# isarandi/metro-pose3d

Measured on AMD Instinct MI355X. Metric: crops/sec (256x256, RN50 stride16), higher is better.
Workload: dtype f16

## Files before the change

### metro_pose3d_amd/csrc/conv_b1.hip

```cpp
#ifndef METRO_WT_STORES
#define METRO_WT_STORES 1
#endif
#include "metro_common.h"
#include "gfx950_prims.h"

namespace metro {

namespace b1 {
constexpr int NPROD = 8, NCONS = 4, NT = 64 * (NPROD + NCONS), TN = 64, K = 64, CB = 256, C2 = 64, NBUF = 3;
constexpr int X_BYTES = TN * 128;
constexpr int OUT_ROW = CB * 2 + 16;
constexpr int OUT_BYTES = TN * OUT_ROW;
constexpr int W1S_ROW = CB * 2 + 16;
static_assert(48 * W1S_ROW <= OUT_BYTES, "W1's stage must fit the second output tile");
template <bool REB>
struct Lay {
    static constexpr int NIN = REB ? 3 : 2;
    static constexpr int X_OFF = 0;
    static constexpr int OUT_OFF = NBUF * NIN * X_BYTES;
    static constexpr int PAR_OFF = OUT_OFF + 2 * OUT_BYTES;
    static constexpr int B3 = 0, BSC = 1024, BB = 2048, B2 = 3072, PRO = 3328, SC2 = 3584, SH2 = 4096, PAR_BYTES = 4608;
    static constexpr int W1T_OFF = PAR_OFF + PAR_BYTES;
    static constexpr int LDS = W1T_OFF + 8 * 64 * 16;
};
// ... 140 lines not shown
#pragma unroll
                    for (int kk = 0; kk < 4; ++kk)
#pragma unroll
                        for (int p = 0; p < 2; ++p) {
                            const half8_t bb = *reinterpret_cast<const half8_t*>(xs + 2 * X_BYTES + p * 4096 + (boff0 ^ (kk << 5)));
                            acc[p] = __builtin_amdgcn_mfma_f32_32x32x16_f16(wbf[kk], bb, acc[p], 0, 0, 0);
                        }
#pragma unroll
                    for (int q = 0; q < 4; ++q) {
                        const floatx4 bv = *reinterpret_cast<const floatx4*>(bias_b_l + wave * 32 + 8 * q + 4 * frag_half);
#pragma unroll
                        for (int p = 0; p < 2; ++p) xsum[p][q] = bias_cvt(acc[p], q, bv) + xsum[p][q];
                    }
                }
#pragma unroll
                for (int p = 0; p < 2; ++p)
#pragma unroll
                    for (int e = 0; e < 16; ++e) acc[p][e] = 0.f;
#pragma unroll
                for (int kk = 0; kk < 4; ++kk)
#pragma unroll
                    for (int p = 0; p < 2; ++p) {
                        const half8_t bf = *reinterpret_cast<const half8_t*>(xs + p * 4096 + (boff0 ^ (kk << 5)));
                        acc[p] = __builtin_amdgcn_mfma_f32_32x32x16_f16(wf[kk], bf, acc[p], 0, 0, 0);
                    }
#pragma unroll
                for (int q = 0; q < 4; ++q) {
                    const int col = wave * 32 + 8 * q + 4 * frag_half;
#pragma unroll
                    for (int p = 0; p < 2; ++p)
                        *reinterpret_cast<half4_t*>(ot + (p * 32 + frag_row) * OUT_ROW + col * 2) = bias_cvt(acc[p], q, b3_r[q]) + xsum[p][q];
                }
            }
            slot = slot == 2 ? 0 : slot + 1;
        }
    } else {
        half8_t w2r[3][8];
        wait_vm_and_barrier<0>();
#pragma unroll
        for (int mt = 0; mt < 3; ++mt)
#pragma unroll
            for (int ks = 0; ks < 8; ++ks) {
                w2r[mt][ks] = *reinterpret_cast<const half8_t*>(smem + L::OUT_OFF + OUT_BYTES + (mt * 16 + (lane & 15)) * W1S_ROW + ks * 64 + (lane >> 4) * 16);
                asm volatile("" : "+v"(w2r[mt][ks]));
            }
        const int wb = wave - NPROD;
        const int px = wb * 16 + (lane & 15), kg = lane >> 4;
        for (int j = 0; j <= T; ++j) {
            wait_lgkm_and_barrier();
            if (j == 0) continue;
            const int tile = t0 + (j - 1) * G;
            const char* ot = smem + L::OUT_OFF + ((j - 1) & 1) * OUT_BYTES;
            const size_t m = (size_t)tile * TN + px;
            bool sub_ok = false;
            size_t sub_row = 0;
            if constexpr (OUTM == 2) {
                const int hw = a.h_out * a.w_out;
                const int m0 = tile * TN + wb * 16;
                const int img = m0 / hw, rem = m0 - img * hw;
                const int hr = (rem >> a.lw_out) - a.sub_off;
                const int wo = ((rem & (a.w_out - 1)) + (lane & 15)) - a.sub_off;
                sub_ok = hr >= 0 && (hr & 1) == 0 && (hr >> 1) < a.h_sub && wo >= 0 && (wo & 1) == 0 && (wo >> 1) < a.w_sub;
                sub_row = ((size_t)img * a.h_sub + (hr >> 1)) * a.w_sub + (wo >> 1);
            }
            floatx4 dacc[4];
#pragma unroll
            for (int mt = 0; mt < 4; ++mt) dacc[mt] = floatx4{0.f, 0.f, 0.f, 0.f};
#pragma unroll
            for (int ks = 0; ks < 8; ++ks) {
                const uint4 v = *reinterpret_cast<const uint4*>(ot + px * OUT_ROW + ks * 64 + kg * 16);
                if constexpr (OUTM == 0) store_out16(a.out + m * CB + ks * 32 + kg * 8, v);
                if constexpr (OUTM == 2) {
                    if (sub_ok) store_out16(a.out_sub + sub_row * CB + ks * 32 + kg * 8, v);
                }
                const half8_t s = *reinterpret_cast<const half8_t*>(par + L::SC2 + (ks * 32 + kg * 8) * 2);
                const half8_t b = *reinterpret_cast<const half8_t*>(par + L::SH2 + (ks * 32 + kg * 8) * 2);
                half8_t pv = *reinterpret_cast<const half8_t*>(&v);
                pv = relu(pv * s + b);
                const half8_t w3 = *reinterpret_cast<const half8_t*>(smem + L::W1T_OFF + (ks * 64 + lane) * 16);
#pragma unroll
                for (int mt = 0; mt < 3; ++mt) dacc[mt] = __builtin_amdgcn_mfma_f32_16x16x32_f16(w2r[mt][ks], pv, dacc[mt], 0, 0, 0);
                dacc[3] = __builtin_amdgcn_mfma_f32_16x16x32_f16(w3, pv, dacc[3], 0, 0, 0);
            }
#pragma unroll
            for (int mt = 0; mt < 4; ++mt) {
                const int co = mt * 16 + kg * 4;
                const floatx4 bv = *reinterpret_cast<const floatx4*>(par + L::B2 + co * 4);
                half4_t hv;
#pragma unroll
                for (int e = 0; e < 4; ++e) hv[e] = (half_t)relu(dacc[mt][e] + bv[e]);
                *reinterpret_cast<half4_t*>(a.out2 + m * C2 + co) = hv;
            }
        }
    }
}

static thread_local int g_b1_force_classic = 0;
void conv_b1_set_form(int classic) { g_b1_force_classic = classic; }
bool classic_forms_forced() { return g_b1_force_classic != 0; }

bool conv_b1_chain_preferred() {
    static const int enabled = tuning_knob("METRO_B1_SPLIT", 1);
    return enabled != 0 && g_b1_force_classic == 0;
}

template <bool REB, int OUTM>
static int launch_b1(B1Args a, hipStream_t stream) {
    if (note_kernel("conv_b1_chain<%s%s>", REB ? "rebuild" : "projsc", OUTM == 1 ? ",noout" : OUTM == 2 ? ",subout" : ""))
        return METRO_OK;
    auto kern = conv_b1_chain_kernel<REB, OUTM>;
    constexpr int lds = b1::Lay<REB>::LDS;
    a.n_tiles = a.m_total / b1::TN;
    static PerDeviceInt cap;
    int grid_cap = 0;
    if (const int st = ensure_dyn_lds_and_grid_cap(reinterpret_cast<const void*>(kern), b1::NT, lds, cap, "conv_b1_chain", 1, &grid_cap))
        return st;
    const int grid = a.n_tiles < grid_cap ? a.n_tiles : grid_cap;
    hipLaunchKernelGGL(kern, dim3(grid), dim3(b1::NT), lds, stream, a);
    return launch_status("conv_b1_chain");
}

int launch_conv_b1_chain(const MetroConvDesc& d, const void* in, const void* w, const float* bias, void* out, hipStream_t stream,
                         const ConvFused& f) {
    const ConvFuse2& f2 = f.next;
    const ConvProjSc& psc = f.psc;
    const ConvRebuild& rb = f.rb;
    B1Args a;
    a.in = static_cast<const half_t*>(in); a.w = static_cast<const half_t*>(w); a.bias = bias;
    a.x_sc = static_cast<const half_t*>(psc.x); a.w_sc = static_cast<const half_t*>(psc.w_sc); a.bias_sc = psc.bias_sc;
    a.pro_scale = static_cast<const half_t*>(psc.pro_scale); a.pro_shift = static_cast<const half_t*>(psc.pro_shift);
    a.in_b = static_cast<const half_t*>(rb.t2_prev); a.w_b = static_cast<const half_t*>(rb.w3_prev); a.bias_b = rb.bias3_prev;
    a.w2 = static_cast<const half_t*>(f2.w2); a.bias2 = f2.bias2;
    a.scale2 = static_cast<const half_t*>(f2.scale2); a.shift2 = static_cast<const half_t*>(f2.shift2);
    a.out = static_cast<half_t*>(out); a.out_sub = static_cast<half_t*>(rb.out_sub); a.out2 = static_cast<half_t*>(f2.out2);
    a.m_total = d.n * d.h_out * d.w_out; a.n_tiles = 0;
    a.h_out = d.h_out; a.w_out = d.w_out; a.lw_out = 0;
    while ((1 << a.lw_out) < d.w_out) ++a.lw_out;
    a.sub_off = rb.sub_off; a.h_sub = rb.h_sub; a.w_sub = rb.w_sub;
    if (f.form == ConvForm::NextRebuild) return rb.out_mode == 2 ? launch_b1<true, 2>(a, stream) : launch_b1<true, 0>(a, stream);
    return rb.out_mode == 1 ? launch_b1<false, 1>(a, stream) : launch_b1<false, 0>(a, stream);
}

}
```

### metro_pose3d_amd/csrc/conv_pw64.hip

```cpp
#include <cstdlib>
#include <type_traits>

#ifndef METRO_WT_STORES
#define METRO_WT_STORES 1
#endif
#include "metro_common.h"
#include "gfx950_prims.h"

namespace metro {

struct Pw64Args {
    const half_t* in;
    const half_t* w;
    const float* bias;
    const half_t* pro_scale;
    const half_t* pro_shift;
    const half_t* residual;
    half_t* out;
    const half_t* w2;
    const float* bias2;
    const half_t* scale2;
    const half_t* shift2;
    half_t* out2;
    const half_t* x_sc;
    const half_t* w_sc;
    const float* bias_sc;
    const half_t* in_b;
    const half_t* w_b;
    const float* bias_b;
    half_t* out_sub;
    int sub_off, h_sub, w_sub, lw_out;
    int m_total, n_tiles;
    int c_out;
    int res_stride, res_off, res_h, res_w, h_out, w_out;
};

namespace pw {
constexpr int NW = 8, NT = 512;
template <int K, int WM, int CB = 256>
struct Lay {
    static constexpr int WN = NW / WM;
    static constexpr int NI = CB / 32 / WM;
    static constexpr int TN = 32 * WN;
    static constexpr int KS = K / 64;
    static constexpr int SL_BYTES = TN * 128;
    static constexpr int X_BYTES = KS * SL_BYTES;
    static constexpr int XI = X_BYTES / 1024 / NW;
    static constexpr int CPR = CB / 8;
    static constexpr int RI = TN * CPR / NT;
    static constexpr int OUT_ROW = CB * 2 + 16;
    static constexpr int OUT_BYTES = TN * OUT_ROW;
    static constexpr int RES_BYTES = TN * CB * 2;
    static constexpr int C2 = CB == 512 ? 128 : 64;
    static constexpr int BIAS2_OFF = CB * 4, PRO_OFF = BIAS2_OFF + 512, BSC_OFF = PRO_OFF + 4 * K, BB_OFF = BSC_OFF + 1024;
    static constexpr int PAR_BYTES = BB_OFF + 1024;
    static constexpr int X_OFF = 0;
    static constexpr int OUT_OFF = X_OFF + 2 * X_BYTES;
    static constexpr int PAR_OFF = OUT_OFF + OUT_BYTES;
    static constexpr int RES_OFF = PAR_OFF + PAR_BYTES;
    static_assert(X_BYTES % (1024 * NW) == 0, "input tile must split evenly over the waves");
    static_assert(NI >= 1 && RI >= 1 && (TN * CPR) % NT == 0, "tile / thread mismatch");
};
template <int K, int WM, bool RES, int MODE2, bool PSC = false, int CB = 256, bool REB = false>
constexpr int lds_bytes() {
    return Lay<K, WM, CB>::RES_OFF + (RES ? 2 * Lay<K, WM, CB>::RES_BYTES : PSC ? (REB ? 4 : 2) * Lay<K, WM, CB>::X_BYTES
                                      : (MODE2 == 1 && K > 64) ? Lay<K, WM, CB>::C2 * (2 * K + 16) + Lay<K, WM, CB>::TN * (2 * Lay<K, WM, CB>::C2 + 16) : 0);
}
}

template <int BASE, int MAXX>
__device__ __forceinline__ void pw_wait_vm_plus(int extra) {
    if constexpr (MAXX == 0) {
        wait_vm<BASE>();
    } else {
        if (extra >= MAXX) wait_vm<BASE + MAXX>();
        else pw_wait_vm_plus<BASE, MAXX - 1>(extra);
    }
}
__device__ __forceinline__ void pw_wait_lgkm2(half8_t& r, half8_t& r2, int n) {
    switch (n) {
        case 0: asm volatile("s_waitcnt lgkmcnt(0)" : "+v"(r), "+v"(r2)); break;
        case 2: asm volatile("s_waitcnt lgkmcnt(2)" : "+v"(r), "+v"(r2)); break;
        case 4: asm volatile("s_waitcnt lgkmcnt(4)" : "+v"(r), "+v"(r2)); break;
        default: asm volatile("s_waitcnt lgkmcnt(6)" : "+v"(r), "+v"(r2)); break;
    }
}

// ... 80 lines not shown
    constexpr bool W2_LDS = MODE2 == 1 && K > 64;
    constexpr bool PREPASS = PRO && W2_LDS;
    constexpr int W2_ROW = 2 * K + 16;
    constexpr int W2_OFF = RES_OFF;
    constexpr int O2_ROW = 2 * C2 + 16, O2_OFF = W2_OFF + C2 * W2_ROW;
    half8_t w2f[MODE2 == 1 && !W2_LDS ? KK : 1];
    if constexpr (MODE2 == 1 && !W2_LDS) {
        if (wave < 4) {
#pragma unroll
            for (int kk = 0; kk < KK; ++kk)
                w2f[kk] = *reinterpret_cast<const half8_t*>(a.w2 + (size_t)(wm * 32 + frag_row) * K + kk * 16 + frag_half * 8);
        }
    }
    if constexpr (W2_LDS) {
        for (int c = tid; c < C2 * (K / 8); c += NT) {
            const int r = c / (K / 8), q = c % (K / 8);
            *reinterpret_cast<uint4*>(smem + W2_OFF + r * W2_ROW + q * 16) = *reinterpret_cast<const uint4*>(a.w2 + (size_t)r * K + q * 8);
        }
    }
    const char* w2l = smem + W2_OFF + (wm * 32 + frag_row) * W2_ROW + frag_half * 16;
    float* bias_l = reinterpret_cast<float*>(smem + PAR_OFF);
    float* bias2_l = reinterpret_cast<float*>(smem + PAR_OFF + L::BIAS2_OFF);
    half_t* pro_l = reinterpret_cast<half_t*>(smem + PAR_OFF + L::PRO_OFF);
    if (tid < CB) bias_l[tid] = a.bias[tid];
    if (MODE2 != 0 && tid < C2) bias2_l[tid] = a.bias2[tid];
    if ((PRO || PSC) && tid < K) { pro_l[tid] = a.pro_scale[tid]; pro_l[K + tid] = a.pro_shift[tid]; }
    float* bias_sc_l = reinterpret_cast<float*>(smem + PAR_OFF + L::BSC_OFF);
    if (PSC && tid < 256) bias_sc_l[tid] = a.bias_sc[tid];
    float* bias_b_l = reinterpret_cast<float*>(smem + PAR_OFF + L::BB_OFF);
    if (REB && tid < 256) bias_b_l[tid] = a.bias_b[tid];
    const int ch = tid & (CPR - 1);
    half8_t sc2 = {}, sh2 = {};
    if constexpr (MODE2 == 2) {
        sc2 = *reinterpret_cast<const half8_t*>(a.scale2 + ch * 8);
        sh2 = *reinterpret_cast<const half8_t*>(a.shift2 + ch * 8);
        if constexpr (!W_STAGED) {
#pragma unroll
            for (int ks = 0; ks < KS2; ++ks)
                w2r[ks] = *reinterpret_cast<const half8_t*>(a.w2 + (size_t)((wave % RG) * 16 + (lane & 15)) * CB + ks * 32 + (lane >> 4) * 8);
        }
    }

    int xrow[XI], xoff[XI];
#pragma unroll
    for (int i = 0; i < XI; ++i) {
        const int q = i * NW + wave;
        xrow[i] = (q % (TN / 8)) * 8 + (lane >> 3);
        xoff[i] = xrow[i] * K + (q / (TN / 8)) * 64 + (((lane & 7) ^ swz<64>(xrow[i])) * 8);
    }
    auto issue_tile = [&](int tile, int buf) {
        const int m0 = tile * TN;
#pragma unroll
        for (int i = 0; i < XI; ++i) {
            const half_t* xs = (m0 + xrow[i] < a.m_total) ? a.in + (size_t)m0 * K + xoff[i] : zero;
            dma16(xs, __builtin_amdgcn_readfirstlane(smem_base + X_OFF + buf * X_BYTES + (i * NW + wave) * 1024));
            if constexpr (PSC) {
                const half_t* ss = (m0 + xrow[i] < a.m_total) ? a.x_sc + (size_t)m0 * K + xoff[i] : zero;
                dma16(ss, __builtin_amdgcn_readfirstlane(smem_base + XS_OFF + buf * X_BYTES + (i * NW + wave) * 1024));
            }
            if constexpr (REB) {
                const half_t* sb = (m0 + xrow[i] < a.m_total) ? a.in_b + (size_t)m0 * K + xoff[i] : zero;
                dma16(sb, __builtin_amdgcn_readfirstlane(smem_base + XB_OFF + buf * X_BYTES + (i * NW + wave) * 1024));
            }
        }
        if constexpr (RES) {
#pragma unroll
            for (int it = 0; it < RI; ++it) {
                const int c = it * NT + tid;
                const int m = m0 + c / CPR;
                size_t rrow = m;
                if constexpr (RSUB) {
                    const int hw = a.h_out * a.w_out;
                    const int img = m / hw, rem = m - img * hw;
                    const int ho = rem / a.w_out, wo = rem - ho * a.w_out;
                    rrow = ((size_t)img * a.res_h + a.res_off + a.res_stride * ho) * a.res_w + a.res_off + a.res_stride * wo;
                }
                const half_t* rs = m < a.m_total ? a.residual + rrow * ldo + (c & (CPR - 1)) * 8 : zero;
                dma16(rs, __builtin_amdgcn_readfirstlane(smem_base + RES_OFF + buf * RES_BYTES + it * 8192 + wave * 1024));
            }
        }
    };

    issue_tile(t, 0);
    constexpr int S2 = MODE2 == 2 ? NTW : (MODE2 == 1 && K > 64) ? 1 : 4;
    constexpr int RS = OUTM == 0 ? RI : 0;
    const bool two = MODE2 == 2 || (MODE2 == 1 && (wave < 4 || K > 64));
    bool prev_full = false;
    int prev_sub = 0;
    for (int it = 0;; ++it, t += G) {
        const int buf = it & 1;
        const int m0 = t * TN;
        if (it == 0 || !prev_full) wait_vm<0>();
        else if constexpr (OUTM == 2) pw_wait_vm_plus<S2, RI>(prev_sub);
        else if (two) wait_vm<RS + S2>();
        else wait_vm<RS>();
        wait_lgkm_and_barrier();
        if (t + G < a.n_tiles) issue_tile(t + G, buf ^ 1);
        prev_full = m0 + TN <= a.m_total;

        if constexpr (PREPASS) {
            static_assert(X_BYTES / 16 == 2 * NT, "two 16-byte chunks of the input tile per thread");
            const int c8 = lane & 7, prow = (wave & 3) * 8 + (lane >> 3);
#pragma unroll
            for (int h = 0; h < 2; ++h) {
                const int sl = (wave >> 2) + 2 * h;
                half8_t* xp = reinterpret_cast<half8_t*>(smem + X_OFF + buf * X_BYTES + sl * SL_BYTES + prow * 128 + ((c8 ^ swz<64>(prow)) << 4));
                const half8_t sc = *reinterpret_cast<const half8_t*>(pro_l + sl * 64 + c8 * 8);
                const half8_t sh = *reinterpret_cast<const half8_t*>(pro_l + K + sl * 64 + c8 * 8);
                *xp = relu(*xp * sc + sh);
            }
            wait_lgkm_and_barrier();
        }
        floatx16 acc[NI], acc2, accs[NI];
#pragma unroll
        for (int e = 0; e < 16; ++e) {
#pragma unroll
            for (int i = 0; i < NI; ++i) { acc[i][e] = 0.f; accs[i][e] = 0.f; }
            acc2[e] = 0.f;
        }
        const char* xl = smem + X_OFF + buf * X_BYTES;
        const int brow = wn * 32 + frag_row;
        half4_t xprev[NI][4];
        if constexpr (REB) {
#pragma unroll
            for (int kk = 0; kk < KK; ++kk) {
                const int chunk = (kk & 3) * 2 + frag_half;
                half8_t bs = *reinterpret_cast<const half8_t*>(smem + XS_OFF + buf * X_BYTES + (kk >> 2) * SL_BYTES + brow * 128 + ((chunk ^ swz<64>(brow)) << 4));
                const half8_t s = *reinterpret_cast<const half8_t*>(pro_l + kk * 16 + frag_half * 8);
                const half8_t b = *reinterpret_cast<const half8_t*>(pro_l + K + kk * 16 + frag_half * 8);
                bs = relu(bs * s + b);
#pragma unroll
                for (int i = 0; i < NI; ++i) accs[i] = __builtin_amdgcn_mfma_f32_32x32x16_f16(wsf[i][kk], bs, accs[i], 0, 0, 0);
            }
#pragma unroll
            for (int i = 0; i < NI; ++i)
#pragma unroll
                for (int q = 0; q < 4; ++q) {
                    const floatx4 bs = *reinterpret_cast<const floatx4*>(bias_sc_l + (wm * NI + i) * 32 + 8 * q + 4 * frag_half);
#pragma unroll
                    for (int e = 0; e < 4; ++e) xprev[i][q][e] = (half_t)(accs[i][4 * q + e] + bs[e]);
                }
            floatx16 accb[NI];
#pragma unroll
            for (int i = 0; i < NI; ++i)
#pragma unroll
                for (int e = 0; e < 16; ++e) accb[i][e] = 0.f;
#pragma unroll
            for (int kk = 0; kk < KK; ++kk) {
                const int chunk = (kk & 3) * 2 + frag_half;
                const half8_t bb = *reinterpret_cast<const half8_t*>(smem + XB_OFF + buf * X_BYTES + (kk >> 2) * SL_BYTES + brow * 128 + ((chunk ^ swz<64>(brow)) << 4));
#pragma unroll
                for (int i = 0; i < NI; ++i) accb[i] = __builtin_amdgcn_mfma_f32_32x32x16_f16(wbf[i][kk], bb, accb[i], 0, 0, 0);
            }
#pragma unroll
            for (int i = 0; i < NI; ++i)
#pragma unroll
                for (int q = 0; q < 4; ++q) {
                    const floatx4 bv = *reinterpret_cast<const floatx4*>(bias_b_l + (wm * NI + i) * 32 + 8 * q + 4 * frag_half);
                    half4_t hb;
#pragma unroll
                    for (int e = 0; e < 4; ++e) hb[e] = (half_t)(accb[i][4 * q + e] + bv[e]);
                    xprev[i][q] = hb + xprev[i][q];
                }
        }
        if constexpr (PREPASS) {
            constexpr int DEPTH = 3;
            unsigned fbase[4];
// ... 95 lines not shown
#pragma unroll
                    for (int e = 0; e < 4; ++e) hs[e] = (half_t)(accs[i][4 * q + e] + bs[e]);
                    hv = hv + hs;
                }
                *reinterpret_cast<half4_t*>(ol + brow * OUT_ROW + col * 2) = hv;
            }
        }
        wait_lgkm_and_barrier();
        const char* rl = smem + RES_OFF + buf * RES_BYTES;
        int img0 = 0, rem0 = 0, now_sub = 0;
        if constexpr (OUTM == 2) {
            const int hw = a.h_out * a.w_out;
            img0 = m0 / hw;
            rem0 = m0 - img0 * hw;
        }
        uint4 vpre[OUTM == 0 ? RI : 1], rpre[OUTM == 0 && RES ? RI : 1];
        if constexpr (OUTM == 0) {
#pragma unroll
            for (int r = 0; r < RI; ++r) {
                const int idx = tid + r * NT;
                vpre[r] = *reinterpret_cast<const uint4*>(ol + (idx / CPR) * OUT_ROW + ch * 16);
                if constexpr (RES) rpre[r] = *reinterpret_cast<const uint4*>(rl + idx * 16);
            }
            __builtin_amdgcn_sched_barrier(0);
        }
        const bool inside = m0 + TN <= a.m_total;
#pragma unroll
        for (int r = 0; r < RI; ++r) {
            const int idx = tid + r * NT;
            const int prow = idx / CPR;
            const int m = m0 + prow;
            uint4 v;
            if constexpr (OUTM == 0) v = vpre[r];
            else v = *reinterpret_cast<const uint4*>(ol + prow * OUT_ROW + ch * 16);
            if constexpr (RES) {
                uint4 rv;
                if constexpr (OUTM == 0) rv = rpre[r];
                else rv = *reinterpret_cast<const uint4*>(rl + idx * 16);
                half2_t* x = reinterpret_cast<half2_t*>(&v);
                const half2_t* rr = reinterpret_cast<const half2_t*>(&rv);
#pragma unroll
                for (int e = 0; e < 4; ++e) x[e] = x[e] + rr[e];
            }
            if constexpr (OUTM == 0) {
                if (inside) store_out16(a.out + (size_t)m * ldo + ch * 8, v);
                else if (m < a.m_total) store_out16(a.out + (size_t)m * ldo + ch * 8, v);
            }
            if constexpr (OUTM == 2) {
                const int hr = ((rem0 + 16 * r) >> a.lw_out) - a.sub_off;
                if (hr >= 0 && (hr & 1) == 0 && (hr >> 1) < a.h_sub) {
                    ++now_sub;
                    const int wo = ((rem0 + prow) & (a.w_out - 1)) - a.sub_off;
                    if (wo >= 0 && (wo & 1) == 0 && (wo >> 1) < a.w_sub)
                        store_out16(a.out_sub + (((size_t)img0 * a.h_sub + (hr >> 1)) * a.w_sub + (wo >> 1)) * CB + ch * 8, v);
                }
            }
            if constexpr (MODE2 == 2) {
                half8_t p = *reinterpret_cast<const half8_t*>(&v);
                p = relu(p * sc2 + sh2);
                *reinterpret_cast<half8_t*>(ol + prow * OUT_ROW + ch * 16) = p;
            }
        }
        if constexpr (W2_LDS) {
            static_assert(TN * (C2 / 8) == NT, "one 16-byte chunk of the second output per thread");
            const int prow2 = tid / (C2 / 8), ch2 = tid % (C2 / 8);
            const uint4 v2 = *reinterpret_cast<const uint4*>(smem + O2_OFF + prow2 * O2_ROW + ch2 * 16);
            if (m0 + prow2 < a.m_total) store_out16(a.out2 + (size_t)(m0 + prow2) * C2 + ch2 * 8, v2);
        }
        if constexpr (MODE2 == 2) {
            wait_lgkm_and_barrier();
            floatx4 dacc[NTW];
#pragma unroll
            for (int j = 0; j < NTW; ++j) dacc[j] = floatx4{0.f, 0.f, 0.f, 0.f};
            const int px0 = (wave / RG) * (NTW * 16);
            const char* bl = ol + (px0 + (lane & 15)) * OUT_ROW + (lane >> 4) * 16;
#pragma unroll
            for (int ks = 0; ks < KS2; ++ks) {
#pragma unroll
                for (int j = 0; j < NTW; ++j) {
                    const half8_t bj = *reinterpret_cast<const half8_t*>(bl + j * 16 * OUT_ROW + ks * 64);
                    dacc[j] = __builtin_amdgcn_mfma_f32_16x16x32_f16(w2r[ks], bj, dacc[j], 0, 0, 0);
                }
            }
            const int co = (wave % RG) * 16 + (lane >> 4) * 4;
            const floatx4 bv = *reinterpret_cast<const floatx4*>(bias2_l + co);
#pragma unroll
            for (int j = 0; j < NTW; ++j) {
                const int m = m0 + px0 + j * 16 + (lane & 15);
                half4_t hv;
#pragma unroll
                for (int e = 0; e < 4; ++e) hv[e] = (half_t)relu(dacc[j][e] + bv[e]);
                if (m < a.m_total) *reinterpret_cast<half4_t*>(a.out2 + (size_t)m * C2 + co) = hv;
            }
        }
        prev_sub = now_sub;
        if (t + G >= a.n_tiles) break;
    }
}

static bool pw_enabled() {
    static const int v = tuning_knob("METRO_PW64", 1);
    return v != 0;
}

static bool b1_map_ok(const MetroConvDesc& d) {
    return (d.h_out * d.w_out) % 64 == 0 && d.w_out >= 16 && (d.w_out & (d.w_out - 1)) == 0;
}

bool conv_pw64_supported(const MetroConvDesc& d, const ConvFused& f) {
    if (!pw_enabled()) return false;
    if (!(d.kh == 1 && d.kw == 1 && d.stride == 1 && d.pad_top == 0 && d.pad_left == 0 && d.in_pix_stride == d.c_in &&
          d.h_in == d.h_out && d.w_in == d.w_out && d.relu == 0 && d.out_dtype == METRO_F16 && d.in_dtype == METRO_F16))
        return false;
    const bool res_plain = d.res_stride == 1 && d.res_offset == 0 && d.res_h == d.h_out && d.res_w == d.w_out;
    const bool res_sub = d.res_stride == 2 && d.res_offset >= 0 && d.res_offset + 2 * (d.h_out - 1) < d.res_h &&
                         d.res_offset + 2 * (d.w_out - 1) < d.res_w;
    if (d.has_residual && !res_plain && !(f.form == ConvForm::Plain && res_sub && d.c_in <= 128)) return false;
    switch (f.form) {
        case ConvForm::Pair: {
            static const int pair256 = tuning_knob("METRO_PW_PAIR256", 1);
            return ((d.c_in == 64 && d.c_out == 320) || (pair256 && !classic_forms_forced() && d.c_in == 256 && d.c_out == 640)) &&
                   d.has_prologue && !d.has_residual && f.pair.relu2 == 1 && 5 * f.pair.c_out2 == d.c_out && f.pair.split == 4 * f.pair.c_out2;
        }
        case ConvForm::Next: {
            static const int next128 = tuning_knob("METRO_PW_NEXT128", 1);
            return ((d.c_in == 64 && d.c_out == 256 && f.next.c2 == 64) ||
                    (next128 && d.c_in == 128 && d.c_out == 512 && res_plain && f.next.c2 == 128)) && !d.has_prologue && d.has_residual;
        }
        case ConvForm::NextProj:
        case ConvForm::NextRebuild:
            return d.c_in == 64 && d.c_out == 256 && !d.has_prologue && !d.has_residual && f.next.c2 == 64 &&
                   (f.form == ConvForm::NextProj || b1_map_ok(d));
        case ConvForm::Plain:
            break;
    }
    if (d.c_in == 64 && d.c_out == 256) return (d.has_prologue != 0) != (d.has_residual != 0);
    static const int maxk = tuning_knob("METRO_PW_MAXK", 512);
    return (d.c_in == 128 || d.c_in == 256 || d.c_in == 512) && d.c_in <= maxk && d.c_out == 4 * d.c_in &&
           !d.has_prologue && d.has_residual;
}

template <int K, int WM, bool PRO, bool RES, int MODE2, bool RSUB = false, bool PSC = false, int CB = 256, bool REB = false, int OUTM = 0>
static int launch_pw(Pw64Args a, hipStream_t stream) {
    if (note_kernel("conv_pw64<k%d,wm%d%s%s%s%s%s%s%s%s>", K, WM, CB == 512 ? ",cb512" : "", PRO ? ",pro" : "", RES ? ",res" : "",
                    MODE2 == 1 ? ",pair" : MODE2 == 2 ? ",next" : "", RSUB ? ",ressub" : "", PSC ? ",projsc" : "", REB ? ",rebuild" : "",
                    OUTM == 1 ? ",noout" : OUTM == 2 ? ",subout" : ""))
        return METRO_OK;
    auto kern = conv_pw64_kernel<K, WM, PRO, RES, MODE2, RSUB, PSC, CB, REB, OUTM>;
    constexpr int lds = pw::lds_bytes<K, WM, RES, MODE2, PSC, CB, REB>();
    a.n_tiles = (a.m_total + pw::Lay<K, WM, CB>::TN - 1) / pw::Lay<K, WM, CB>::TN;
    static PerDeviceInt cap;
    int grid_cap = 0;
    if (const int st = ensure_dyn_lds_and_grid_cap(reinterpret_cast<const void*>(kern), pw::NT, lds, cap, "conv_pw64",
                                                   tuning_knob("METRO_PW64_BPC", 0) , &grid_cap))
        return st;
    const int halves = a.c_out / CB;
    int grid = a.n_tiles * halves < grid_cap ? a.n_tiles * halves : grid_cap;
    grid -= grid % halves;
    hipLaunchKernelGGL(kern, dim3(grid), dim3(pw::NT), lds, stream, a);
    return launch_status("conv_pw64");
}

int launch_conv_pw64(const MetroConvDesc& d, const void* in, const void* w, const float* bias, const void* ps,
                     const void* pb, const void* res, void* out, hipStream_t stream, const ConvFused& f) {
    const ConvRebuild& rb = f.rb;
    if ((f.form == ConvForm::NextRebuild || (f.form == ConvForm::NextProj && rb.out_mode == 1)) && !rb.classic &&
        conv_b1_chain_preferred() && b1_map_ok(d))
        return launch_conv_b1_chain(d, in, w, bias, out, stream, f);
    Pw64Args a;
    a.in = static_cast<const half_t*>(in);
    a.w = static_cast<const half_t*>(w);
    a.bias = bias;
    a.pro_scale = static_cast<const half_t*>(ps);
    a.pro_shift = static_cast<const half_t*>(pb);
    a.residual = d.has_residual ? static_cast<const half_t*>(res) : nullptr;
// ... 46 lines not shown
```

### metro_pose3d_amd/csrc/conv_pws.hip

```cpp
#include "metro_common.h"
#include "gfx950_prims.h"

namespace metro {

struct PwsArgs {
    const half_t* in;
    const half_t* w;
    const float* bias;
    const half_t* residual;
    half_t* out;
    int m_total, n_tiles, c_out;
};

namespace pws {
constexpr int NW = 8, NT = 512, TN = 32, CB = 256, NBUF = 3;
constexpr int T_ROW = 80;
constexpr int T_BYTES = TN * T_ROW;
constexpr int R_BYTES = TN * 64;
template <int K>
struct Lay {
    static constexpr int KS = K / 64;
    static constexpr int SL_BYTES = TN * 128;
    static constexpr int X_BYTES = KS * SL_BYTES;
    static constexpr int NX = X_BYTES / 1024 / NW;
    static constexpr int X_OFF = 0;
    static constexpr int T_OFF = NBUF * X_BYTES;
    static constexpr int BIAS_OFF = T_OFF + NW * (T_BYTES + R_BYTES);
    static constexpr int LDS = BIAS_OFF + CB * 4;
    static_assert(X_BYTES % (1024 * NW) == 0, "operand tile must split evenly over the waves");
};
}

template <int K>
__global__ __launch_bounds__(pws::NT) void conv_pws_kernel(PwsArgs a) {
    using namespace pws;
    using L = Lay<K>;
    constexpr int KK = K / 16, NX = L::NX, X_BYTES = L::X_BYTES, SL_BYTES = L::SL_BYTES;
    extern __shared__ __attribute__((aligned(16))) char smem[];
    const unsigned smem_base = lds_offset_of(smem);
    const int tid = threadIdx.x;
    const int lane = tid & 63;
    const int wave = __builtin_amdgcn_readfirstlane(tid >> 6);
    const int frag_row = lane & 31, frag_half = lane >> 5;

    const int halves = a.c_out / CB;
    const int G = gridDim.x / halves;
    int half, t0;
    if ((gridDim.x & 7) == 0 && ((gridDim.x >> 3) % halves) == 0) {
        const int xcd = blockIdx.x & 7, j = blockIdx.x >> 3;
        half = j % halves;
        t0 = xcd * ((gridDim.x >> 3) / halves) + j / halves;
    } else {
        half = blockIdx.x % halves;
        t0 = blockIdx.x / halves;
    }
    if (t0 >= a.n_tiles) return;
    const int T = (a.n_tiles - t0 + G - 1) / G;
    const int ldo = a.c_out;
    const int co0 = half * CB + wave * 32;

    half8_t wf[KK];
    static_assert(L::BIAS_OFF >= NW * W_STAGE_BYTES, "the staging scratch must not reach the bias block");
    load_w_frags_staged<K>(a.w + (size_t)co0 * K, wf, smem + wave * W_STAGE_BYTES, lane);
#pragma unroll
    for (int kk = 0; kk < KK; ++kk) asm volatile("" : "+v"(wf[kk]));
    float* bias_l = reinterpret_cast<float*>(smem + L::BIAS_OFF);
    if (tid < CB) bias_l[tid] = a.bias[half * CB + tid];

    int xoff[NX];
#pragma unroll
    for (int i = 0; i < NX; ++i) {
        const int q = i * NW + wave;
        const int row = (q & 3) * 8 + (lane >> 3);
        xoff[i] = row * K + (q >> 2) * 64 + (((lane & 7) ^ swz<64>(row)) * 8);
    }
    auto issue_x = [&](int tile, int slot) {
        const half_t* src = a.in + (size_t)tile * TN * K;
#pragma unroll
        for (int i = 0; i < NX; ++i)
            dma16(src + xoff[i], __builtin_amdgcn_readfirstlane(smem_base + L::X_OFF + slot * X_BYTES + (i * NW + wave) * 1024));
    };
    char* tw = smem + L::T_OFF + wave * (T_BYTES + R_BYTES);
    const unsigned rw_lds = smem_base + L::T_OFF + wave * (T_BYTES + R_BYTES) + T_BYTES;
    const int rpx = lane >> 2, rch = lane & 3;
    auto issue_res = [&](int tile) {
        const half_t* src = a.residual + ((size_t)tile * TN + rpx) * ldo + co0 + rch * 8;
        dma16(src, __builtin_amdgcn_readfirstlane(rw_lds));
        dma16(src + (size_t)16 * ldo, __builtin_amdgcn_readfirstlane(rw_lds + 1024));
    };
    const int boff0 = frag_row * 128 + ((frag_half ^ swz<64>(frag_row)) << 4);

    wait_vm_and_barrier<0>();
    floatx4 bv[4];
#pragma unroll
    for (int q = 0; q < 4; ++q) bv[q] = *reinterpret_cast<const floatx4*>(bias_l + wave * 32 + 8 * q + 4 * frag_half);
    issue_x(t0, 0);
    if (T > 1) issue_x(t0 + G, 1);
    if (T > 1) wait_vm<NX>();
    else wait_vm<0>();
    if (wave >= 4) wait_lgkm_and_barrier();

    int slot = 0;
    for (int j = 0; j < T; ++j) {
        const int tile = t0 + j * G;
        wait_lgkm_and_barrier();
        issue_res(tile);
        if (j + 2 < T) issue_x(t0 + (j + 2) * G, slot >= 1 ? slot - 1 : 2);
        floatx16 acc;
#pragma unroll
        for (int e = 0; e < 16; ++e) acc[e] = 0.f;
        constexpr int DEPTH = 8;
        unsigned fbase[4];
#pragma unroll
        for (int c = 0; c < 4; ++c) fbase[c] = smem_base + L::X_OFF + slot * X_BYTES + (boff0 ^ (c << 5));
        half8_t fr[DEPTH];
#pragma unroll
        for (int kk = 0; kk < DEPTH; ++kk)
            asm volatile("ds_read_b128 %0, %1 offset:%2" : "=v"(fr[kk]) : "v"(fbase[kk & 3]), "n"((kk >> 2) * SL_BYTES));
#pragma unroll
        for (int kk = 0; kk < KK; ++kk) {
            if (KK - 1 - kk >= DEPTH - 1) asm volatile("s_waitcnt lgkmcnt(%1)" : "+v"(fr[kk % DEPTH]) : "n"(DEPTH - 1));
            else wait_lgkm_dyn(fr[kk % DEPTH], KK - 1 - kk);
            acc = __builtin_amdgcn_mfma_f32_32x32x16_f16(wf[kk], fr[kk % DEPTH], acc, 0, 0, 0);
            if (kk + DEPTH < KK)
                asm volatile("ds_read_b128 %0, %1 offset:%2" : "=v"(fr[kk % DEPTH]) : "v"(fbase[(kk + DEPTH) & 3]), "n"(((kk + DEPTH) >> 2) * SL_BYTES));
        }
        if (j + 2 < T) wait_vm<NX>();
        else wait_vm<0>();
        wait_lgkm_and_barrier();
#pragma unroll
        for (int q = 0; q < 4; ++q)
            *reinterpret_cast<half4_t*>(tw + frag_row * T_ROW + (8 * q + 4 * frag_half) * 2) = bias_cvt(acc, q, bv[q]);
        asm volatile("s_waitcnt lgkmcnt(0)" ::: "memory");
#pragma unroll
        for (int it = 0; it < 2; ++it) {
            const int px = it * 16 + rpx;
            uint4 v = *reinterpret_cast<const uint4*>(tw + px * T_ROW + rch * 16);
            const uint4 rv = *reinterpret_cast<const uint4*>(tw + T_BYTES + it * 1024 + lane * 16);
            half8_t x = __builtin_bit_cast(half8_t, v);
            x = x + __builtin_bit_cast(half8_t, rv);
            store_out16(a.out + ((size_t)tile * TN + px) * ldo + co0 + rch * 8, __builtin_bit_cast(uint4, x));
        }
        slot = slot == 2 ? 0 : slot + 1;
    }
    if (wave < 4) wait_lgkm_and_barrier();
}

bool conv_pws_supported(const MetroConvDesc& d) {
    static const int enabled = tuning_knob("METRO_PWS", 1);
    if (!enabled || classic_forms_forced()) return false;
    if (!(d.kh == 1 && d.kw == 1 && d.stride == 1 && d.pad_top == 0 && d.pad_left == 0 && d.in_pix_stride == d.c_in &&
          d.h_in == d.h_out && d.w_in == d.w_out && d.relu == 0 && d.out_dtype == METRO_F16 && d.in_dtype == METRO_F16))
        return false;
    const bool res_plain = d.has_residual && d.res_stride == 1 && d.res_offset == 0 && d.res_h == d.h_out && d.res_w == d.w_out;
    const long m = (long)d.n * d.h_out * d.w_out;
    if (!((d.c_in == 256 || d.c_in == 512) && d.c_out == 4 * d.c_in && !d.has_prologue && res_plain && m % pws::TN == 0)) return false;
    static const int k256_max_items = tuning_knob("METRO_PWS_K256_MAX_ITEMS", 16);
    if (d.c_in == 512) return true;
    const long items = (m / pws::TN) * (d.c_out / pws::CB);
    return items <= (long)k256_max_items * 256;
}

template <int K>
static int launch_pws(PwsArgs a, hipStream_t stream) {
    if (note_kernel("conv_pws<k%d,res>", K)) return METRO_OK;
    auto kern = conv_pws_kernel<K>;
    constexpr int lds = pws::Lay<K>::LDS;
    a.n_tiles = a.m_total / pws::TN;
    static PerDeviceInt cap;
    int grid_cap = 0;
    if (const int st = ensure_dyn_lds_and_grid_cap(reinterpret_cast<const void*>(kern), pws::NT, lds, cap, "conv_pws", 1, &grid_cap)) return st;
    const int halves = a.c_out / pws::CB;
    int grid = a.n_tiles * halves < grid_cap ? a.n_tiles * halves : grid_cap;
    grid -= grid % halves;
    hipLaunchKernelGGL(kern, dim3(grid), dim3(pws::NT), lds, stream, a);
    return launch_status("conv_pws");
}

int launch_conv_pws(const MetroConvDesc& d, const void* in, const void* w, const float* bias, const void* res, void* out, hipStream_t stream) {
    if (!conv_pws_supported(d)) { set_error("conv_pws: unsupported layer"); return METRO_ERR_UNSUPPORTED; }
    PwsArgs a;
    a.in = static_cast<const half_t*>(in); a.w = static_cast<const half_t*>(w); a.bias = bias;
    a.residual = static_cast<const half_t*>(res); a.out = static_cast<half_t*>(out);
    a.m_total = d.n * d.h_out * d.w_out; a.n_tiles = 0; a.c_out = d.c_out;
    if (d.c_in == 512) return launch_pws<512>(a, stream);
    return launch_pws<256>(a, stream);
}

}
```

### metro_pose3d_amd/csrc/gfx950_prims.h

```cpp
#pragma once
#include <hip/hip_runtime.h>
#include <type_traits>

#if defined(__HIP_DEVICE_COMPILE__) && !defined(__gfx950__)
#error "the metro kernels are written for gfx950 (CDNA4) only: build with --offload-arch=gfx950"
#endif

namespace metro {

typedef _Float16 half_t;
typedef _Float16 half2_t __attribute__((ext_vector_type(2)));
typedef _Float16 half4_t __attribute__((ext_vector_type(4)));
typedef _Float16 half8_t __attribute__((ext_vector_type(8)));
typedef float floatx4 __attribute__((ext_vector_type(4)));
typedef float floatx16 __attribute__((ext_vector_type(16)));
typedef __attribute__((address_space(3))) void lds_void_t;

__device__ __forceinline__ unsigned lds_offset_of(const void* p) {
    return (unsigned)(size_t)(lds_void_t*)p;
}

static __device__ __attribute__((aligned(16))) unsigned int g_zero_page[4];

__device__ __forceinline__ void dma16(const void* gsrc, unsigned lds_addr) {
    asm volatile(
        "s_mov_b32 m0, %1\n\t"
        "s_nop 0\n\t"
        "global_load_lds_dwordx4 %0, off"
        :
        : "v"(gsrc), "s"(lds_addr));
}
template <int LDS_IMM>
__device__ __forceinline__ void dma16s(const void* sbase, unsigned voff, unsigned lds_base) {
    asm volatile(
        "s_add_u32 m0, %2, %3\n\t"
        "s_nop 0\n\t"
        "global_load_lds_dwordx4 %0, %1"
        :
        : "v"(voff), "s"(sbase), "s"(lds_base), "n"(LDS_IMM)
        : "scc");
}

template <int N>
__device__ __forceinline__ void wait_vm() {
    asm volatile("s_waitcnt vmcnt(%0)" ::"n"(N) : "memory");
}
template <int N>
__device__ __forceinline__ void wait_vm_and_barrier() {
    asm volatile("s_waitcnt vmcnt(%0) lgkmcnt(0)\n\ts_barrier" ::"n"(N) : "memory");
}
__device__ __forceinline__ void wait_lgkm_and_barrier() {
    asm volatile("s_waitcnt lgkmcnt(0)\n\ts_barrier" ::: "memory");
}
__device__ __forceinline__ void wait_lgkm_dyn(half8_t& r, int n) {
    switch (n) {
        case 0: asm volatile("s_waitcnt lgkmcnt(0)" : "+v"(r)); break;
        case 1: asm volatile("s_waitcnt lgkmcnt(1)" : "+v"(r)); break;
        case 2: asm volatile("s_waitcnt lgkmcnt(2)" : "+v"(r)); break;
        case 3: asm volatile("s_waitcnt lgkmcnt(3)" : "+v"(r)); break;
        case 4: asm volatile("s_waitcnt lgkmcnt(4)" : "+v"(r)); break;
        case 5: asm volatile("s_waitcnt lgkmcnt(5)" : "+v"(r)); break;
        default: asm volatile("s_waitcnt lgkmcnt(6)" : "+v"(r)); break;
    }
}

template <int BK>
__device__ __forceinline__ int swz(int row) {
    static_assert(BK == 64 || BK == 32, "128- or 64-byte rows");
    return BK == 64 ? (row >> 1) & 7 : (row >> 2) & 3;
}

__device__ __forceinline__ half4_t bias_cvt(const floatx16& acc, int q, const floatx4& bv) {
    typedef float f32x2 __attribute__((ext_vector_type(2)));
    typedef unsigned int u32x2 __attribute__((ext_vector_type(2)));
    f32x2 lo = {acc[4 * q], acc[4 * q + 1]}, hi = {acc[4 * q + 2], acc[4 * q + 3]};
    const f32x2 blo = {bv[0], bv[1]}, bhi = {bv[2], bv[3]};
    asm("v_pk_add_f32 %0, %1, %2" : "=v"(lo) : "v"(lo), "v"(blo));
    asm("v_pk_add_f32 %0, %1, %2" : "=v"(hi) : "v"(hi), "v"(bhi));
    u32x2 r;
    asm("v_cvt_pk_f16_f32 %0, %1, %2" : "=v"(r.x) : "v"(lo.x), "v"(lo.y));
    asm("v_cvt_pk_f16_f32 %0, %1, %2" : "=v"(r.y) : "v"(hi.x), "v"(hi.y));
    return __builtin_bit_cast(half4_t, r);
}

template <typename T>
__device__ __forceinline__ T relu(T v) {
    return __builtin_elementwise_maximum(v, T{});
}

template <typename T>
__device__ __forceinline__ T opaque_copy(T v) {
    asm volatile("" : "+v"(v));
    return v;
}

template <int N, int I = 0, class F>
__device__ __forceinline__ void static_for(F&& f) {
    if constexpr (I < N) {
        f(std::integral_constant<int, I>{});
        static_for<N, I + 1>(f);
    }
}

}
```

### metro_pose3d_amd/csrc/metro_common.h

```cpp
#pragma once
#include <hip/hip_runtime.h>
#include <cstdarg>
#include <cstdint>
#include <cstdio>
#include <cstdlib>

#include "../../include/metro_hip.h"

namespace metro {

void set_error(const char* fmt, ...);
const char* get_error();

#define METRO_CHECK_ARG(cond, ...)                  \
    do {                                            \
        if (!(cond)) {                              \
            ::metro::set_error(__VA_ARGS__);        \
            return METRO_ERR_INVALID_ARG;           \
        }                                           \
    } while (0)

#define METRO_HIP_CHECK(expr)                                                              \
    do {                                                                                   \
        hipError_t _e = (expr);                                                            \
        if (_e != hipSuccess) {                                                            \
            ::metro::set_error("%s failed: %s (%s:%d)", #expr, hipGetErrorString(_e),      \
                               __FILE__, __LINE__);                                        \
            return METRO_ERR_HIP;                                                          \
        }                                                                                  \
    } while (0)

inline int tuning_knob(const char* name, int dflt) {
#ifdef METRO_TUNING_KNOBS
    const char* e = getenv(name);
    return e ? atoi(e) : dflt;
#else
    (void)name;
    return dflt;
#endif
}

struct KernelNotes { int mode; char ids[1024]; };
KernelNotes& kernel_notes();
bool note_kernel(const char* fmt, ...) __attribute__((format(printf, 1, 2)));

typedef unsigned int metro_u32x4 __attribute__((ext_vector_type(4)));
#ifndef METRO_WT_STORES
#define METRO_WT_STORES 0
#endif
__device__ __forceinline__ void store_out16(void* p, uint4 v) {
#if METRO_WT_STORES
    const metro_u32x4 w = {v.x, v.y, v.z, v.w};
    asm volatile("global_store_dwordx4 %0, %1, off sc1\n\ts_nop 1" ::"v"(p), "v"(w));
#else
    *reinterpret_cast<uint4*>(p) = v;
#endif
}

constexpr int W_STAGE_ROW = 272;
constexpr int W_STAGE_BYTES = 32 * W_STAGE_ROW;
template <int K, typename Frag>
__device__ __forceinline__ void load_w_frags_staged(const _Float16* __restrict__ rows , Frag* wf ,
                                                    char* scratch , int lane) {
    static_assert(K % 128 == 0 || K == 64, "whole 256-byte row pieces (K = 64: one 128-byte piece)");
    constexpr int PIECE = K >= 128 ? 128 : 64;
    constexpr int LPR = PIECE / 8;
    constexpr int RPI = 64 / LPR;
    const int lr = lane / LPR, lc = lane % LPR;
    const int fr = lane & 31, fh = lane >> 5;
#pragma unroll
    for (int c = 0; c < K / PIECE; ++c) {
#pragma unroll
        for (int j = 0; j < 32 / RPI; ++j)
            *reinterpret_cast<uint4*>(scratch + (j * RPI + lr) * W_STAGE_ROW + lc * 16) =
                *reinterpret_cast<const uint4*>(rows + (size_t)(j * RPI + lr) * K + c * PIECE + lc * 8);
        __builtin_amdgcn_wave_barrier();
#pragma unroll
        for (int k8 = 0; k8 < PIECE / 16; ++k8)
            wf[c * (PIECE / 16) + k8] = *reinterpret_cast<const Frag*>(scratch + fr * W_STAGE_ROW + k8 * 32 + fh * 16);
        __builtin_amdgcn_wave_barrier();
    }
}

template <int K, typename Frag>
__device__ __forceinline__ void load_w_frags16_staged(const _Float16* __restrict__ rows, Frag* wf , char* scratch, int lane) {
    static_assert(K % 128 == 0, "whole 256-byte row pieces");
    const int lr = lane >> 4, lc = lane & 15;
#pragma unroll
    for (int c = 0; c < K / 128; ++c) {
#pragma unroll
        for (int j = 0; j < 4; ++j)
            *reinterpret_cast<uint4*>(scratch + (j * 4 + lr) * W_STAGE_ROW + lc * 16) =
                *reinterpret_cast<const uint4*>(rows + (size_t)(j * 4 + lr) * K + c * 128 + lc * 8);
        __builtin_amdgcn_wave_barrier();
#pragma unroll
        for (int k4 = 0; k4 < 4; ++k4)
            wf[c * 4 + k4] = *reinterpret_cast<const Frag*>(scratch + (lane & 15) * W_STAGE_ROW + k4 * 64 + (lane >> 4) * 16);
        __builtin_amdgcn_wave_barrier();
    }
}

constexpr int METRO_MAX_DEVICES = 64;
struct PerDeviceInt { int v[METRO_MAX_DEVICES]; };

inline int current_device_slot(int* slot) {
    int dev = 0;
    const hipError_t e = hipGetDevice(&dev);
    if (e != hipSuccess || dev < 0 || dev >= METRO_MAX_DEVICES) {
        set_error("hipGetDevice: %s (device %d; at most %d devices per process)", hipGetErrorString(e), dev, METRO_MAX_DEVICES);
        return METRO_ERR_HIP;
    }
    *slot = dev;
    return METRO_OK;
}

inline int ensure_dyn_lds(const void* kern, int bytes, PerDeviceInt& done, const char* what) {
    int slot = 0;
    const int st = current_device_slot(&slot);
    if (st) return st;
    if (done.v[slot]) return METRO_OK;
    const hipError_t e = hipFuncSetAttribute(kern, hipFuncAttributeMaxDynamicSharedMemorySize, bytes);
    if (e != hipSuccess) {
        set_error("hipFuncSetAttribute(%s, %d B of LDS, device %d): %s", what, bytes, slot, hipGetErrorString(e));
        return METRO_ERR_HIP;
    }
    done.v[slot] = 1;
    return METRO_OK;
}

inline int ensure_dyn_lds_and_grid_cap(const void* kern, int threads, int bytes, PerDeviceInt& cap, const char* what,
                                       int max_blocks_per_cu, int* grid_cap) {
    int slot = 0;
    int st = current_device_slot(&slot);
    if (st) return st;
    if (cap.v[slot] == 0) {
        const hipError_t e = hipFuncSetAttribute(kern, hipFuncAttributeMaxDynamicSharedMemorySize, bytes);
        if (e != hipSuccess) {
            set_error("hipFuncSetAttribute(%s, %d B of LDS, device %d): %s", what, bytes, slot, hipGetErrorString(e));
            return METRO_ERR_HIP;
        }
// ... 241 lines not shown
```

Before: 49170.

## Widen second-output stores via permlane16 swap and defer pws output stores

In the b1 chain and pw64 MODE2==2 paths, pairs of half4 results from adjacent lane groups are exchanged with permlane16_swap so that each lane issues one 16-byte store instead of two 8-byte stores. This halves the store count, and the vmcnt wait budget S2 is updated to match. In pws, output stores for K=256 now use the sc1 write-through variant and are deferred by one tile, so they overlap the next tile's MFMA work, with the wait counts adjusted accordingly. The changes add lane-exchange instructions, hold the deferred values in extra registers, and the revised wait counts carry correctness risk.

```diff
diff --git a/metro_pose3d_amd/csrc/conv_b1.hip b/metro_pose3d_amd/csrc/conv_b1.hip
--- a/metro_pose3d_amd/csrc/conv_b1.hip
+++ b/metro_pose3d_amd/csrc/conv_b1.hip
@@ -246,14 +246,17 @@
                 for (int mt = 0; mt < 3; ++mt) dacc[mt] = __builtin_amdgcn_mfma_f32_16x16x32_f16(w2r[mt][ks], pv, dacc[mt], 0, 0, 0);
                 dacc[3] = __builtin_amdgcn_mfma_f32_16x16x32_f16(w3, pv, dacc[3], 0, 0, 0);
             }
+            half4_t hv[4];
 #pragma unroll
             for (int mt = 0; mt < 4; ++mt) {
-                const int co = mt * 16 + kg * 4;
-                const floatx4 bv = *reinterpret_cast<const floatx4*>(par + L::B2 + co * 4);
-                half4_t hv;
-#pragma unroll
-                for (int e = 0; e < 4; ++e) hv[e] = (half_t)relu(dacc[mt][e] + bv[e]);
-                *reinterpret_cast<half4_t*>(a.out2 + m * C2 + co) = hv;
+                const floatx4 bv = *reinterpret_cast<const floatx4*>(par + L::B2 + (mt * 16 + kg * 4) * 4);
+#pragma unroll
+                for (int e = 0; e < 4; ++e) hv[mt][e] = (half_t)relu(dacc[mt][e] + bv[e]);
+            }
+#pragma unroll
+            for (int u = 0; u < 2; ++u) {
+                const uint4 v = join_kg_pairs(hv[2 * u], hv[2 * u + 1]);
+                store_out16(a.out2 + m * C2 + (2 * u + (kg & 1)) * 16 + (kg >> 1) * 8, v);
             }
         }
     }
diff --git a/metro_pose3d_amd/csrc/conv_pw64.hip b/metro_pose3d_amd/csrc/conv_pw64.hip
--- a/metro_pose3d_amd/csrc/conv_pw64.hip
+++ b/metro_pose3d_amd/csrc/conv_pw64.hip
@@ -3,6 +3,9 @@
 
 #ifndef METRO_WT_STORES
 #define METRO_WT_STORES 1
+#endif
+#ifndef METRO_PW64_OUT2_WT
+#define METRO_PW64_OUT2_WT 0
 #endif
 #include "metro_common.h"
 #include "gfx950_prims.h"
@@ -249,7 +252,8 @@
     };
 
     issue_tile(t, 0);
-    constexpr int S2 = MODE2 == 2 ? NTW : (MODE2 == 1 && K > 64) ? 1 : 4;
+    static_assert(MODE2 != 2 || NTW % 2 == 0, "the second output's lane exchange pairs the pixel groups of a wave");
+    constexpr int S2 = MODE2 == 2 ? NTW / 2 : (MODE2 == 1 && K > 64) ? 1 : 4;
     constexpr int RS = OUTM == 0 ? RI : 0;
     const bool two = MODE2 == 2 || (MODE2 == 1 && (wave < 4 || K > 64));
     bool prev_full = false;
@@ -511,15 +515,19 @@
                     dacc[j] = __builtin_amdgcn_mfma_f32_16x16x32_f16(w2r[ks], bj, dacc[j], 0, 0, 0);
                 }
             }
-            const int co = (wave % RG) * 16 + (lane >> 4) * 4;
-            const floatx4 bv = *reinterpret_cast<const floatx4*>(bias2_l + co);
-#pragma unroll
-            for (int j = 0; j < NTW; ++j) {
-                const int m = m0 + px0 + j * 16 + (lane & 15);
-                half4_t hv;
-#pragma unroll
-                for (int e = 0; e < 4; ++e) hv[e] = (half_t)relu(dacc[j][e] + bv[e]);
-                if (m < a.m_total) *reinterpret_cast<half4_t*>(a.out2 + (size_t)m * C2 + co) = hv;
+            const int kg = lane >> 4;
+            const floatx4 bv = *reinterpret_cast<const floatx4*>(bias2_l + (wave % RG) * 16 + kg * 4);
+            half4_t hv[NTW];
+#pragma unroll
+            for (int j = 0; j < NTW; ++j)
+#pragma unroll
+                for (int e = 0; e < 4; ++e) hv[j][e] = (half_t)relu(dacc[j][e] + bv[e]);
+            const int co = (wave % RG) * 16 + (kg >> 1) * 8;
+#pragma unroll
+            for (int u = 0; u < NTW / 2; ++u) {
+                const uint4 v = join_kg_pairs(hv[2 * u], hv[2 * u + 1]);
+                const int m = m0 + px0 + (2 * u + (kg & 1)) * 16 + (lane & 15);
+                if (m < a.m_total) store_out16_as<METRO_PW64_OUT2_WT != 0>(a.out2 + (size_t)m * C2 + co, v);
             }
         }
         prev_sub = now_sub;
diff --git a/metro_pose3d_amd/csrc/conv_pws.hip b/metro_pose3d_amd/csrc/conv_pws.hip
--- a/metro_pose3d_amd/csrc/conv_pws.hip
+++ b/metro_pose3d_amd/csrc/conv_pws.hip
@@ -1,3 +1,9 @@
+#ifndef METRO_PWS_WT_K256
+#define METRO_PWS_WT_K256 1
+#endif
+#ifndef METRO_PWS_WT_K512
+#define METRO_PWS_WT_K512 0
+#endif
 #include "metro_common.h"
 #include "gfx950_prims.h"
 
@@ -36,6 +42,8 @@
     using namespace pws;
     using L = Lay<K>;
     constexpr int KK = K / 16, NX = L::NX, X_BYTES = L::X_BYTES, SL_BYTES = L::SL_BYTES;
+    constexpr bool WT = (K == 512 ? METRO_PWS_WT_K512 : METRO_PWS_WT_K256) != 0;
+    constexpr bool DEFER = WT;
     extern __shared__ __attribute__((aligned(16))) char smem[];
     const unsigned smem_base = lds_offset_of(smem);
     const int tid = threadIdx.x;
@@ -100,12 +108,24 @@
     else wait_vm<0>();
     if (wave >= 4) wait_lgkm_and_barrier();
 
+    constexpr int KEPT = DEFER ? 2 : 0;
+    uint4 kept[2] = {};
+    half_t* const out_l = a.out + (size_t)rpx * ldo + co0 + rch * 8;
+    auto store_kept = [&](int tile) {
+        asm volatile("" ::: "memory");
+#pragma unroll
+        for (int it = 0; it < 2; ++it) store_out16_as<WT>(out_l + ((size_t)tile * TN + it * 16) * ldo, kept[it]);
+    };
+
     int slot = 0;
     for (int j = 0; j < T; ++j) {
         const int tile = t0 + j * G;
         wait_lgkm_and_barrier();
         issue_res(tile);
         if (j + 2 < T) issue_x(t0 + (j + 2) * G, slot >= 1 ? slot - 1 : 2);
+        if constexpr (DEFER) {
+            if (j > 0) store_kept(tile - G);
+        }
         floatx16 acc;
 #pragma unroll
         for (int e = 0; e < 16; ++e) acc[e] = 0.f;
@@ -125,8 +145,13 @@
             if (kk + DEPTH < KK)
                 asm volatile("ds_read_b128 %0, %1 offset:%2" : "=v"(fr[kk % DEPTH]) : "v"(fbase[(kk + DEPTH) & 3]), "n"(((kk + DEPTH) >> 2) * SL_BYTES));
         }
-        if (j + 2 < T) wait_vm<NX>();
-        else wait_vm<0>();
+        if (j + 2 < T) {
+            if (j > 0) wait_vm<NX + KEPT>();
+            else wait_vm<NX>();
+        } else {
+            if (j > 0) wait_vm<KEPT>();
+            else wait_vm<0>();
+        }
         wait_lgkm_and_barrier();
 #pragma unroll
         for (int q = 0; q < 4; ++q)
@@ -139,10 +164,12 @@
             const uint4 rv = *reinterpret_cast<const uint4*>(tw + T_BYTES + it * 1024 + lane * 16);
             half8_t x = __builtin_bit_cast(half8_t, v);
             x = x + __builtin_bit_cast(half8_t, rv);
-            store_out16(a.out + ((size_t)tile * TN + px) * ldo + co0 + rch * 8, __builtin_bit_cast(uint4, x));
-        }
+            kept[it] = __builtin_bit_cast(uint4, x);
+        }
+        if constexpr (!DEFER) store_kept(tile);
         slot = slot == 2 ? 0 : slot + 1;
     }
+    if constexpr (DEFER) store_kept(t0 + (T - 1) * G);
     if (wave < 4) wait_lgkm_and_barrier();
 }
 
diff --git a/metro_pose3d_amd/csrc/gfx950_prims.h b/metro_pose3d_amd/csrc/gfx950_prims.h
--- a/metro_pose3d_amd/csrc/gfx950_prims.h
+++ b/metro_pose3d_amd/csrc/gfx950_prims.h
@@ -83,6 +83,14 @@
     return __builtin_bit_cast(half4_t, r);
 }
 
+__device__ __forceinline__ uint4 join_kg_pairs(half4_t p0, half4_t p1) {
+    typedef unsigned int u32x2 __attribute__((ext_vector_type(2)));
+    const u32x2 a = __builtin_bit_cast(u32x2, p0), b = __builtin_bit_cast(u32x2, p1);
+    const u32x2 x = __builtin_amdgcn_permlane16_swap(a.x, b.x, false, false);
+    const u32x2 y = __builtin_amdgcn_permlane16_swap(a.y, b.y, false, false);
+    return uint4{x.x, y.x, x.y, y.y};
+}
+
 template <typename T>
 __device__ __forceinline__ T relu(T v) {
     return __builtin_elementwise_maximum(v, T{});
diff --git a/metro_pose3d_amd/csrc/metro_common.h b/metro_pose3d_amd/csrc/metro_common.h
--- a/metro_pose3d_amd/csrc/metro_common.h
+++ b/metro_pose3d_amd/csrc/metro_common.h
@@ -48,14 +48,16 @@
 #ifndef METRO_WT_STORES
 #define METRO_WT_STORES 0
 #endif
-__device__ __forceinline__ void store_out16(void* p, uint4 v) {
-#if METRO_WT_STORES
-    const metro_u32x4 w = {v.x, v.y, v.z, v.w};
-    asm volatile("global_store_dwordx4 %0, %1, off sc1\n\ts_nop 1" ::"v"(p), "v"(w));
-#else
-    *reinterpret_cast<uint4*>(p) = v;
-#endif
-}
+template <bool WT>
+__device__ __forceinline__ void store_out16_as(void* p, uint4 v) {
+    if constexpr (WT) {
+        const metro_u32x4 w = {v.x, v.y, v.z, v.w};
+        asm volatile("global_store_dwordx4 %0, %1, off sc1\n\ts_nop 1" ::"v"(p), "v"(w));
+    } else {
+        *reinterpret_cast<uint4*>(p) = v;
+    }
+}
+__device__ __forceinline__ void store_out16(void* p, uint4 v) { store_out16_as<METRO_WT_STORES != 0>(p, v); }
 
 constexpr int W_STAGE_ROW = 272;
 constexpr int W_STAGE_BYTES = 32 * W_STAGE_ROW;
```

After: 49340 (median of 6 runs). Within noise of the previous version (+0.3%).
